# GradientSpaces/LivingScenes

Hardware: AMD Instinct MI355X
Metric: object-instances/sec (encode+match+register), N=1024 pts (higher is better)
Workload: dtype f32 (GEMM products as two-piece f16 splits on the f16 matrix cores, fp32 accumulate: as accurate against fp64 as an fp32 FMA chain)

## Files before the change

### livingscenes_amd/csrc/edge.hip

```cpp
#include "ls_launch.h"
#include "ls_device.h"

namespace ls {

constexpr int EK = 16;

__global__ __launch_bounds__(256) void edge_l0_kernel(const float* __restrict__ pts, const int32_t* __restrict__ knn,
                                                      const float* __restrict__ w0, int N, int Co, float oms,
                                                      float* __restrict__ out, int total) {
    const int lane = threadIdx.x & 63, wave = threadIdx.x >> 6;
    const int sub = lane >> 5, o = lane & 31;
    int pid = (xcd_remap(blockIdx.x, gridDim.x) * 4 + wave) * 2 + sub;
    const bool live = pid < total;
    if (!live) pid = total - 1;
    const int b = pid / N;
    const float* P = pts + (size_t)b * N * 3;
    const float cx = pts[(size_t)pid * 3 + 0], cy = pts[(size_t)pid * 3 + 1], cz = pts[(size_t)pid * 3 + 2];
    const float inv = 1.0f / fmaxf(sqrtf(cx * cx + cy * cy + cz * cz), 1e-12f);
    const float ax = cx * inv, ay = cy * inv, az = cz * inv;
    const int32_t* ki = knn + (size_t)pid * EK;
    __shared__ __attribute__((aligned(16))) float l_edge[4][2][EK][8];
    if (o < EK) {
        const int r = ki[o];
        const float nx = P[(size_t)r * 3 + 0], ny = P[(size_t)r * 3 + 1], nz = P[(size_t)r * 3 + 2];
        float* le = l_edge[wave][sub][o];
        *reinterpret_cast<float4*>(le) = make_float4(ay * nz - az * ny, az * nx - ax * nz, ax * ny - ay * nx, nx - cx);
        *reinterpret_cast<float2*>(le + 4) = make_float2(ny - cy, nz - cz);
    }
    __builtin_amdgcn_s_waitcnt(0xc07f);
    __builtin_amdgcn_wave_barrier();
    for (int c0 = 0; c0 < Co; c0 += 32) {
        const int oc = c0 + o;
        const bool on = oc < Co;
        const int ow = on ? oc : 0;
        const float a0 = w0[0 * Co + ow], a1 = w0[1 * Co + ow], a2 = w0[2 * Co + ow];
        const float d0 = w0[3 * Co + ow], d1 = w0[4 * Co + ow], d2 = w0[5 * Co + ow];
        const float yc0 = a2 * cx, yc1 = a2 * cy, yc2 = a2 * cz, kc0 = d2 * cx, kc1 = d2 * cy, kc2 = d2 * cz;
        float s0 = 0.f, s1 = 0.f, s2 = 0.f;
#pragma unroll 4
        for (int k = 0; k < EK; ++k) {
            const float4 e0 = *reinterpret_cast<const float4*>(l_edge[wave][sub][k]);
            const float2 e1 = *reinterpret_cast<const float2*>(l_edge[wave][sub][k] + 4);
            const float crx = e0.x, cry = e0.y, crz = e0.z, dx = e0.w, dy = e1.x, dz = e1.y;
            float y0 = __builtin_fmaf(a0, crx, __builtin_fmaf(a1, dx, yc0)), y1 = __builtin_fmaf(a0, cry, __builtin_fmaf(a1, dy, yc1)),
                  y2 = __builtin_fmaf(a0, crz, __builtin_fmaf(a1, dz, yc2));
            const float k0 = __builtin_fmaf(d0, crx, __builtin_fmaf(d1, dx, kc0)), k1 = __builtin_fmaf(d0, cry, __builtin_fmaf(d1, dy, kc1)),
                        k2 = __builtin_fmaf(d0, crz, __builtin_fmaf(d1, dz, kc2));
            vn_act(y0, y1, y2, k0, k1, k2, oms);
            s0 += y0; s1 += y1; s2 += y2;
        }
        if (live && on) {
            float* op = out + (size_t)pid * 3 * Co + oc;
            op[0] = s0 * (1.0f / EK); op[Co] = s1 * (1.0f / EK); op[2 * Co] = s2 * (1.0f / EK);
        }
    }
}

__global__ __launch_bounds__(256) void edge_pool_kernel(const float* __restrict__ T, int ldt, const float* __restrict__ Tq, int ldq,
                                                        int NQ, int q_via_rows, const int32_t* __restrict__ knn,
                                                        const int32_t* __restrict__ dst_rows, int Nd, int Ns, int Co,
                                                        float oms, float* __restrict__ out, int total) {
    const int lane = threadIdx.x & 63, wave = threadIdx.x >> 6;
    const int lpp = Co <= 32 ? 32 : 64;
    const int ppw = 64 / lpp;
    const int sub = lane / lpp, ol = lane % lpp;
    int pid = (xcd_remap(blockIdx.x, gridDim.x) * 4 + wave) * ppw + sub;
    const bool live = pid < total;
    if (!live) pid = total - 1;
    const int b = pid / Nd;
    const int drow = (dst_rows && q_via_rows) ? dst_rows[pid] : (pid % Nd);
    const float* Tb = T + (size_t)b * Ns * 3 * ldt;
    const float* Td = Tq + ((size_t)b * NQ + drow) * 3 * ldq;
    const int32_t* ki = knn + (size_t)pid * EK;
    for (int c0 = 0; c0 < Co; c0 += lpp) {
        const int oc = c0 + ol;
        const bool on = oc < Co;
        const int ow = on ? oc : 0;
        float ql[3], qd[3];
#pragma unroll
        for (int x = 0; x < 3; ++x) { ql[x] = Td[x * ldq + ow]; qd[x] = Td[x * ldq + Co + ow]; }
        float s0 = 0.f, s1 = 0.f, s2 = 0.f;
#pragma unroll 4
        for (int k = 0; k < EK; ++k) {
            const float* Tr = Tb + (size_t)ki[k] * 3 * ldt;
            float y0 = Tr[ow] + ql[0], y1 = Tr[ldt + ow] + ql[1], y2 = Tr[2 * ldt + ow] + ql[2];
            const float k0 = Tr[Co + ow] + qd[0], k1 = Tr[ldt + Co + ow] + qd[1], k2 = Tr[2 * ldt + Co + ow] + qd[2];
            vn_act(y0, y1, y2, k0, k1, k2, oms);
            s0 += y0; s1 += y1; s2 += y2;
        }
        if (live && on) {
            float* op = out + (size_t)pid * 3 * Co + oc;
            op[0] = s0 * (1.0f / EK); op[Co] = s1 * (1.0f / EK); op[2 * Co] = s2 * (1.0f / EK);
        }
    }
}

__global__ __launch_bounds__(256) void edge_attn_kernel(const float* __restrict__ T, int ldt, const float* __restrict__ Tq, int ldq,
                                                        int NQ, int q_via_rows, const int32_t* __restrict__ knn,
                                                        const int32_t* __restrict__ dst_rows, int Nd, int Ns, int Co,
                                                        float oms, float inv_sqrt_dk, float* __restrict__ out, int total) {
    extern __shared__ __attribute__((aligned(16))) float smem[];
    const int lane = threadIdx.x & 63, wave = threadIdx.x >> 6;
    const int nh = Co / 16;
    const int per_wave = 3 * Co + 2 * nh * EK;
    float* lq = smem + (size_t)wave * per_wave;
    float* lscore = lq + 3 * Co;
    float* latt = lscore + nh * EK;
    int pid = xcd_remap(blockIdx.x, gridDim.x) * 4 + wave;
    const bool live = pid < total;
    if (!live) pid = total - 1;
    const int b = pid / Nd;
    const int drow = (dst_rows && q_via_rows) ? dst_rows[pid] : (pid % Nd);
    const float* Tb = T + (size_t)b * Ns * 3 * ldt;
    const float* Td = Tq + ((size_t)b * NQ + drow) * 3 * ldq;
    const int32_t* ki = knn + (size_t)pid * EK;
    int nbr[EK];
#pragma unroll
    for (int k = 0; k < EK; ++k) nbr[k] = ki[k];

    float ssq = 0.f;
    for (int c0 = 0; c0 < Co; c0 += 64) {
        const int oc = c0 + lane;
        if (oc < Co) {
            float y0 = Td[4 * Co + oc], y1 = Td[ldq + 4 * Co + oc], y2 = Td[2 * ldq + 4 * Co + oc];
            const float k0 = Td[5 * Co + oc], k1 = Td[ldq + 5 * Co + oc], k2 = Td[2 * ldq + 5 * Co + oc];
            vn_act(y0, y1, y2, k0, k1, k2, oms);
            lq[oc] = y0; lq[Co + oc] = y1; lq[2 * Co + oc] = y2;
            ssq += y0 * y0 + y1 * y1 + y2 * y2;
        }
    }
    const float inv_q = 1.0f / fmaxf(sqrtf(wave_sum(ssq)), 1e-12f);
    __syncthreads();

    float ssk[EK];
#pragma unroll
    for (int k = 0; k < EK; ++k) ssk[k] = 0.f;
    for (int c0 = 0; c0 < Co; c0 += 64) {
        const int oc = c0 + lane;
        const bool on = oc < Co;
        const int ow = on ? oc : 0;
        float ql[3], qd[3], qv[3];
#pragma unroll
        for (int x = 0; x < 3; ++x) {
            ql[x] = Td[x * ldq + 2 * Co + ow];
            qd[x] = Td[x * ldq + 3 * Co + ow];
            qv[x] = lq[x * Co + ow];
        }
#pragma unroll
        for (int k = 0; k < EK; ++k) {
            const float* Tr = Tb + (size_t)nbr[k] * 3 * ldt;
            float y0 = Tr[2 * Co + ow] + ql[0], y1 = Tr[ldt + 2 * Co + ow] + ql[1], y2 = Tr[2 * ldt + 2 * Co + ow] + ql[2];
            const float k0 = Tr[3 * Co + ow] + qd[0], k1 = Tr[ldt + 3 * Co + ow] + qd[1], k2 = Tr[2 * ldt + 3 * Co + ow] + qd[2];
            vn_act(y0, y1, y2, k0, k1, k2, oms);
            float a = y0 * qv[0] + y1 * qv[1] + y2 * qv[2];
            float s2 = y0 * y0 + y1 * y1 + y2 * y2;
            if (!on) { a = 0.f; s2 = 0.f; }
            ssk[k] += s2;
            const float hs = row16_sum(a);
            if (on && (lane & 15) == 0) lscore[(oc >> 4) * EK + k] = hs;
        }
    }
    float my_invk = 0.f;
#pragma unroll
    for (int k = 0; k < EK; ++k) {
        const float f = 1.0f / fmaxf(sqrtf(wave_sum(ssk[k])), 1e-12f);
        if ((lane & 15) == k) my_invk = f;
    }
    __syncthreads();
    for (int e0 = 0; e0 < nh * EK; e0 += 64) {
        const int e = e0 + lane;
        const bool on = e < nh * EK;
        float v = on ? lscore[e] * inv_q * my_invk * inv_sqrt_dk : -INFINITY;
        const float m = row16_max(v);
        const float ex = on ? expf(v - m) : 0.f;
        const float s = row16_sum(ex);
        if (on) latt[e] = ex / s;
    }
    __syncthreads();

    for (int c0 = 0; c0 < Co; c0 += 64) {
        const int oc = c0 + lane;
        const bool on = oc < Co;
        const int ow = on ? oc : 0;
        float ql[3], qd[3];
#pragma unroll
        for (int x = 0; x < 3; ++x) { ql[x] = Td[x * ldq + ow]; qd[x] = Td[x * ldq + Co + ow]; }
        const float* aw = latt + (ow >> 4) * EK;
        float s0 = 0.f, s1 = 0.f, s2 = 0.f;
#pragma unroll
        for (int k = 0; k < EK; ++k) {
            const float* Tr = Tb + (size_t)nbr[k] * 3 * ldt;
            float y0 = Tr[ow] + ql[0], y1 = Tr[ldt + ow] + ql[1], y2 = Tr[2 * ldt + ow] + ql[2];
            const float k0 = Tr[Co + ow] + qd[0], k1 = Tr[ldt + Co + ow] + qd[1], k2 = Tr[2 * ldt + Co + ow] + qd[2];
            vn_act(y0, y1, y2, k0, k1, k2, oms);
            const float w = aw[k];
            s0 += w * y0; s1 += w * y1; s2 += w * y2;
        }
        if (live && on) {
            float* op = out + (size_t)pid * 3 * Co + oc;
            op[0] = s0; op[Co] = s1; op[2 * Co] = s2;
        }
    }
}


template <int LPP>
__global__ __launch_bounds__(256) __attribute__((amdgpu_waves_per_eu(4))) void edge_pool_v4_kernel(const float* __restrict__ T, int ldt, const float* __restrict__ Tq, int ldq, int NQ,
                                                           int q_via_rows, const int32_t* __restrict__ knn, const int32_t* __restrict__ dst_rows,
                                                           int Nd, int Ns, float oms, float* __restrict__ out, int total) {
    constexpr int PPW = 64 / LPP, Co = 4 * LPP;
    const int lane = threadIdx.x & 63, wave = threadIdx.x >> 6;
    const int sub = lane / LPP, ll = lane % LPP;
    int pid = (xcd_remap(blockIdx.x, gridDim.x) * 4 + wave) * PPW + sub;
    const bool live = pid < total;
    if (!live) pid = total - 1;
    const int b = pid / Nd;
    const int drow = (dst_rows && q_via_rows) ? dst_rows[pid] : (pid % Nd);
    const float* Td = Tq + ((size_t)b * NQ + drow) * 3 * ldq;
    const int c4 = ll * 4;
    int nb[EK];
    {
        const int4* kp = reinterpret_cast<const int4*>(knn + (size_t)pid * EK);
#pragma unroll
        for (int u = 0; u < EK / 4; ++u) { const int4 v = kp[u]; nb[4 * u] = v.x; nb[4 * u + 1] = v.y; nb[4 * u + 2] = v.z; nb[4 * u + 3] = v.w; }
    }
    const F43 ql = ld43(Td + c4, ldq), qd = ld43(Td + Co + c4, ldq);
    F43 acc;
    acc.x = acc.y = acc.z = make_float4(0.f, 0.f, 0.f, 0.f);
    const unsigned row_bytes = 3u * (unsigned)ldt * 4u, lane_off = (unsigned)c4 * 4u, inst_row = (unsigned)b * (unsigned)Ns;
    auto ldrow = [&](unsigned off, int col) {
        asm volatile("" : "+v"(off));
        F43 r;
        r.x = *reinterpret_cast<const float4*>(reinterpret_cast<const char*>(T + col) + off);
        r.y = *reinterpret_cast<const float4*>(reinterpret_cast<const char*>(T + ldt + col) + off);
        r.z = *reinterpret_cast<const float4*>(reinterpret_cast<const char*>(T + 2 * ldt + col) + off);
        return r;
    };
    constexpr int DP = 2;
    F43 py[DP], pd[DP];
#pragma unroll
    for (int d = 0; d < DP; ++d) { const unsigned o = __umul24(inst_row + (unsigned)nb[d], row_bytes) + lane_off; py[d] = ldrow(o, 0); pd[d] = ldrow(o, Co); }
#pragma unroll
    for (int k = 0; k < EK; ++k) {
        F43 y = py[k % DP], kd = pd[k % DP];
        if (k + DP < EK) {
            unsigned o = __umul24(inst_row + (unsigned)nb[k + DP], row_bytes) + lane_off;
            py[k % DP] = ldrow(o, 0); pd[k % DP] = ldrow(o, Co);
        }
        asm volatile("" ::: "memory");
        __builtin_amdgcn_sched_barrier(0);
        y = add43(y, ql);
        kd = add43(kd, qd);
        act43(y, kd, oms);
        acc = add43(acc, y);
        asm volatile("" : "+v"(acc.x.x), "+v"(acc.x.y), "+v"(acc.x.z), "+v"(acc.x.w), "+v"(acc.y.x), "+v"(acc.y.y), "+v"(acc.y.z), "+v"(acc.y.w), "+v"(acc.z.x), "+v"(acc.z.y), "+v"(acc.z.z), "+v"(acc.z.w) :: "memory");
        __builtin_amdgcn_sched_barrier(0);
    }
    if (live) {
        float* op = out + (size_t)pid * 3 * Co + c4;
        const float s = 1.0f / EK;
        *reinterpret_cast<float4*>(op) = make_float4(acc.x.x * s, acc.x.y * s, acc.x.z * s, acc.x.w * s);
        *reinterpret_cast<float4*>(op + Co) = make_float4(acc.y.x * s, acc.y.y * s, acc.y.z * s, acc.y.w * s);
        *reinterpret_cast<float4*>(op + 2 * Co) = make_float4(acc.z.x * s, acc.z.y * s, acc.z.z * s, acc.z.w * s);
    }
}

template <int LPP>
__device__ __forceinline__ void attn_colsum(float (*l_score)[256], const float4& ox, const float4& oy, const float4& oz, bool live, int tid, float* __restrict__ cp) {
    constexpr int PPW = 64 / LPP, PW = 4 * PPW, Co = 4 * LPP;
    const float z = live ? 1.f : 0.f;
    l_score[0][tid] = ox.x * z; l_score[1][tid] = ox.y * z; l_score[2][tid] = ox.z * z; l_score[3][tid] = ox.w * z;
    l_score[4][tid] = oy.x * z; l_score[5][tid] = oy.y * z; l_score[6][tid] = oy.z * z; l_score[7][tid] = oy.w * z;
    l_score[8][tid] = oz.x * z; l_score[9][tid] = oz.y * z; l_score[10][tid] = oz.z * z; l_score[11][tid] = oz.w * z;
    __syncthreads();
    for (int col = tid; col < 3 * Co; col += 256) {
        const int ax = col / Co, c = col - ax * Co;
        const float* sp = &l_score[ax * 4 + (c & 3)][c >> 2];
        float a = 0.f;
#pragma unroll
        for (int pw = 0; pw < PW; ++pw) a += sp[(pw / PPW) * 64 + (pw % PPW) * LPP];
        cp[col] = a;
    }
}

template <int LPP, int NCH>
__global__ __launch_bounds__(256) void edge_attn_v4_kernel(const float* __restrict__ T, int ldt, const float* __restrict__ Tq, int ldq,
                                                           int NQ, int q_via_rows, const int32_t* __restrict__ knn,
                                                           const int32_t* __restrict__ dst_rows, int Nd, int Ns, int Co,
                                                           float oms, float inv_sqrt_dk, float* __restrict__ out, int total,
                                                           float* __restrict__ rowmax, float* __restrict__ colsum) {
    constexpr int PPW = 64 / LPP;
    __shared__ float l_score[NCH][EK][256];
    __shared__ float l_ssk[EK][256];
    const int tid = threadIdx.x, lane = tid & 63, wave = tid >> 6;
    const int sub = lane / LPP, ll = lane % LPP;
    int pid = (xcd_remap(blockIdx.x, gridDim.x) * 4 + wave) * PPW + sub;
    const bool live = pid < total;
    if (!live) pid = total - 1;
    const int b = pid / Nd;
    const int drow = (dst_rows && q_via_rows) ? dst_rows[pid] : (pid % Nd);
    const float* Tb = T + (size_t)b * Ns * 3 * ldt;
    const float* Td = Tq + ((size_t)b * NQ + drow) * 3 * ldq;
    const int32_t* ki = knn + (size_t)pid * EK;

    F43 qf[NCH];
    float ssq = 0.f;
#pragma unroll
    for (int ch = 0; ch < NCH; ++ch) {
        const int c4 = (ch * LPP + ll) * 4;
        qf[ch] = ld43(Td + 4 * Co + c4, ldq);
        const F43 kd = ld43(Td + 5 * Co + c4, ldq);
        act43(qf[ch], kd, oms);
        ssq += dot43(qf[ch], qf[ch]);
    }
    const float inv_q = inv_fro(group_sum<LPP>(ssq));

#pragma unroll
    for (int ch = 0; ch < NCH; ++ch) {
        const int c4 = (ch * LPP + ll) * 4;
        const F43 ql = ld43(Td + 2 * Co + c4, ldq), qd = ld43(Td + 3 * Co + c4, ldq);
#pragma unroll 2
        for (int k = 0; k < EK; ++k) {
            const float* Tr = Tb + (size_t)ki[k] * 3 * ldt;
            F43 y = add43(ld43(Tr + 2 * Co + c4, ldt), ql);
            const F43 kd = add43(ld43(Tr + 3 * Co + c4, ldt), qd);
            act43(y, kd, oms);
            const float s2 = dot43(y, y);
            l_ssk[k][tid] = (ch == 0) ? s2 : l_ssk[k][tid] + s2;
            l_score[ch][k][tid] = quad_sum(dot43(y, qf[ch]));
        }
    }
    float mx[NCH], sum[NCH];
#pragma unroll
    for (int ch = 0; ch < NCH; ++ch) { mx[ch] = -INFINITY; sum[ch] = 0.f; }
#pragma unroll 4
    for (int k = 0; k < EK; ++k) {
        const float invk = inv_fro(group_sum<LPP>(l_ssk[k][tid]));
#pragma unroll
        for (int ch = 0; ch < NCH; ++ch) {
            const float v = l_score[ch][k][tid] * inv_q * invk * inv_sqrt_dk;
            l_score[ch][k][tid] = v;
            mx[ch] = fmaxf(mx[ch], v);
        }
    }
#pragma unroll
    for (int ch = 0; ch < NCH; ++ch) {
#pragma unroll 4
        for (int k = 0; k < EK; ++k) {
            const float ex = expf(l_score[ch][k][tid] - mx[ch]);
            l_score[ch][k][tid] = ex;
            sum[ch] += ex;
        }
    }

    float rmx = 0.f, rmy = 0.f, rmz = 0.f;
#pragma unroll
    for (int ch = 0; ch < NCH; ++ch) {
        const int c4 = (ch * LPP + ll) * 4;
        const F43 ql = ld43(Td + c4, ldq), qd = ld43(Td + Co + c4, ldq);
        F43 acc;
        acc.x = acc.y = acc.z = make_float4(0.f, 0.f, 0.f, 0.f);
#pragma unroll 2
        for (int k = 0; k < EK; ++k) {
            const float* Tr = Tb + (size_t)ki[k] * 3 * ldt;
            F43 y = add43(ld43(Tr + c4, ldt), ql);
            const F43 kd = add43(ld43(Tr + Co + c4, ldt), qd);
            act43(y, kd, oms);
            const float w = l_score[ch][k][tid];
            fma43(acc, w, y);
        }
        const float inv = 1.0f / sum[ch];
        const float4 ox = make_float4(acc.x.x * inv, acc.x.y * inv, acc.x.z * inv, acc.x.w * inv);
        const float4 oy = make_float4(acc.y.x * inv, acc.y.y * inv, acc.y.z * inv, acc.y.w * inv);
        const float4 oz = make_float4(acc.z.x * inv, acc.z.y * inv, acc.z.z * inv, acc.z.w * inv);
        if (live) {
            float* op = out + (size_t)pid * 3 * Co + c4;
            *reinterpret_cast<float4*>(op) = ox;
            *reinterpret_cast<float4*>(op + Co) = oy;
            *reinterpret_cast<float4*>(op + 2 * Co) = oz;
        }
        rmx = fmaxf(rmx, amax_f4(ox)); rmy = fmaxf(rmy, amax_f4(oy)); rmz = fmaxf(rmz, amax_f4(oz));
        if constexpr (NCH == 1) {
            if (colsum) attn_colsum<LPP>(l_score[0], ox, oy, oz, live, tid, colsum + (size_t)xcd_remap(blockIdx.x, gridDim.x) * 3 * Co);
        }
    }
    if (rowmax) {
        rmx = group_max<LPP>(rmx); rmy = group_max<LPP>(rmy); rmz = group_max<LPP>(rmz);
        if (live && ll == 0) { float* rp = rowmax + (size_t)pid * 3; rp[0] = rmx; rp[1] = rmy; rp[2] = rmz; }
    }
}


__global__ __launch_bounds__(64) void edge_presplit_wq_kernel(const float* __restrict__ W, int rows, int Cin, int KS, uint4* __restrict__ planes,
                                                               float* __restrict__ winv) {
    const int tile = blockIdx.x / KS, ks = blockIdx.x % KS, lane = threadIdx.x;
    const int n = tile * 32 + (lane & 31), k = ks * 16 + 8 * (lane >> 5);
    const float* wr = W + (size_t)min(n, rows - 1) * Cin;
    float am = 0.f;
    for (int c = 0; c < Cin; ++c) am = fmaxf(am, fabsf(wr[c]));
    float sc, inv;
    pow2_scale(am, sc, inv);
    if (ks == 0 && lane < 32 && n < rows) winv[n] = inv;
    __attribute__((aligned(16))) float v[8];
#pragma unroll
    for (int c = 0; c < 8; ++c) v[c] = wr[k + c] * sc;
    f16x8_t h, l;
    split8_f16(v, h, l);
    planes[((size_t)blockIdx.x * 2) * 64 + lane] = __builtin_bit_cast(uint4, h);
    planes[((size_t)blockIdx.x * 2 + 1) * 64 + lane] = __builtin_bit_cast(uint4, l);
}
static size_t edge_wq_plane_count(int Co, int Cin) { return (size_t)(6 * Co / 32) * (Cin / 16) * 2 * 64; }
size_t edge_wq_planes_bytes(int Co, int Cin) { return edge_wq_plane_count(Co, Cin) * sizeof(uint4) + (size_t)6 * Co * sizeof(float); }
int edge_presplit_wq_launch(const float* Wq, int Co, int Cin, void* planes, hipStream_t st) {
    hipLaunchKernelGGL(edge_presplit_wq_kernel, dim3((6 * Co / 32) * (Cin / 16)), dim3(64), 0, st, Wq, 6 * Co, Cin, Cin / 16, (uint4*)planes,
                       (float*)((uint4*)planes + edge_wq_plane_count(Co, Cin)));
    LS_LAUNCH_CHECK();
    return LS_OK;
}

template <int LPP, int CIN>
__global__ __launch_bounds__(256) __attribute__((amdgpu_waves_per_eu(3))) void edge_attn_fq_kernel(const float* __restrict__ T, int ldt, const float* __restrict__ cur,
                                                           const uint4* __restrict__ Wp, const int32_t* __restrict__ knn,
                                                           const int32_t* __restrict__ dst_rows, int Nd, int Ns, float oms, float inv_sqrt_dk,
                                                           float* __restrict__ out, int total, float* __restrict__ rowmax, float* __restrict__ colsum) {
    constexpr int PPW = 64 / LPP, PW = 4 * PPW, ROWS = 3 * PW, MT = (ROWS + 31) / 32, Co = LPP * 4, SC = 2 * Co, NT = SC / 32, SLD = SC + 4,
                  KS = CIN / 16, ASTR = CIN * 2 + 16;
    static_assert(MT * NT == 8, "two output tiles per wave");
    __shared__ float l_score[EK][256];
    __shared__ __attribute__((aligned(16))) float slab[ROWS * SLD];
    __shared__ __attribute__((aligned(16))) char a_pl[2][MT * 32 * ASTR];
    __shared__ int a_inv[MT * 32];
    const float* __restrict__ winv = reinterpret_cast<const float*>(Wp + (size_t)(6 * Co / 32) * KS * 128);
    const int tid = threadIdx.x, lane = tid & 63, wave = tid >> 6;
    const int sub = lane / LPP, ll = lane % LPP;
    const int pid0 = xcd_remap(blockIdx.x, gridDim.x) * PW;
    const int pwl = wave * PPW + sub;
    int pid = pid0 + pwl;
    const bool live = pid < total;
    if (!live) pid = total - 1;
    const int b = pid / Nd;
    const float* Tb = T + (size_t)b * Ns * 3 * ldt;
    const int32_t* ki = knn + (size_t)pid * EK;
    const int c4 = ll * 4;

    uint4 wfh[2][KS], wfl[2][KS];
    auto qload = [&](int cb) {
        const uint4* wt = Wp + (size_t)(cb / 32) * KS * 128 + lane;
#pragma unroll
        for (int u = 0; u < (MT == 2 ? 1 : 2); ++u) {
            const int nt = MT == 2 ? wave : wave + 4 * u;
#pragma unroll
            for (int ks = 0; ks < KS; ++ks) {
                wfh[u][ks] = wt[((size_t)(nt * KS + ks) * 2) * 64];
                wfl[u][ks] = wt[((size_t)(nt * KS + ks) * 2 + 1) * 64];
            }
        }
    };
    qload(4 * Co);
    for (int c = tid; c < MT * 32 * (CIN / 4); c += 256) {
        const int r = c / (CIN / 4), kq = c - r * (CIN / 4);
        uint2 h = make_uint2(0u, 0u), l = make_uint2(0u, 0u);
        float4 v = make_float4(0.f, 0.f, 0.f, 0.f);
        if (r < ROWS) {
            const int pw = r / 3, x = r - 3 * pw;
            const int pa = min(pid0 + pw, total - 1), ba = pa / Nd;
            const int sp = dst_rows ? dst_rows[pa] : pa - ba * Nd;
            v = *reinterpret_cast<const float4*>(cur + (((size_t)ba * Ns + sp) * 3 + x) * CIN + kq * 4);
        }
        {
            float am = fmaxf(fmaxf(fabsf(v.x), fabsf(v.y)), fmaxf(fabsf(v.z), fabsf(v.w)));
            am = max8(am);
            if constexpr (CIN == 64) am = dpp_max<0x140>(am);
            float sc, inv;
            pow2_scale(am, sc, inv);
            if (kq == 0) a_inv[r] = pow2_e(inv);
            split2_f16_pair(f32x2_t{v.x * sc, v.y * sc}, h.x, l.x);
            split2_f16_pair(f32x2_t{v.z * sc, v.w * sc}, h.y, l.y);
        }
        *reinterpret_cast<uint2*>(&a_pl[0][r * ASTR + kq * 8]) = h;
        *reinterpret_cast<uint2*>(&a_pl[1][r * ASTR + kq * 8]) = l;
    }
    __syncthreads();

    auto qmma = [&](int cb) {
        __builtin_amdgcn_sched_barrier(0);
#pragma unroll
        for (int u = 0; u < 2; ++u) {
            const int mt = MT == 2 ? u : 0, nt = MT == 2 ? wave : wave + 4 * u;
            const int aoff = (32 * mt + (lane & 31)) * ASTR + (lane >> 5) * 16;
            f32x16_t acc;
#pragma unroll
            for (int r = 0; r < 16; ++r) acc[r] = 0.f;
#pragma unroll
            for (int ks = 0; ks < KS; ++ks) {
                const f16x8_t ah = __builtin_bit_cast(f16x8_t, *reinterpret_cast<const uint4*>(&a_pl[0][aoff + ks * 32]));
                const f16x8_t al = __builtin_bit_cast(f16x8_t, *reinterpret_cast<const uint4*>(&a_pl[1][aoff + ks * 32]));
                const f16x8_t bh = __builtin_bit_cast(f16x8_t, wfh[MT == 2 ? 0 : u][ks]);
                const f16x8_t bl = __builtin_bit_cast(f16x8_t, wfl[MT == 2 ? 0 : u][ks]);
                acc = __builtin_amdgcn_mfma_f32_32x32x16_f16(al, bh, acc, 0, 0, 0);
                acc = __builtin_amdgcn_mfma_f32_32x32x16_f16(ah, bh, acc, 0, 0, 0);
                acc = __builtin_amdgcn_mfma_f32_32x32x16_f16(ah, bl, acc, 0, 0, 0);
            }
            const int row0 = 32 * mt + 4 * (lane >> 5);
            float* sp = slab + row0 * SLD + 32 * nt + (lane & 31);
            const int ce = pow2_e(winv[cb + 32 * nt + (lane & 31)]);
#pragma unroll
            for (int r = 0; r < 16; ++r) {
                const int dr = (r & 3) + 8 * (r >> 2);
                if (row0 + dr < ROWS) sp[dr * SLD] = scale_pow2(acc[r], a_inv[row0 + dr] + ce);
            }
        }
    };
    const float* srow = slab + 3 * pwl * SLD + c4;
    auto lds43 = [&](int col) {
        F43 r;
        r.x = *reinterpret_cast<const float4*>(srow + col);
        r.y = *reinterpret_cast<const float4*>(srow + SLD + col);
        r.z = *reinterpret_cast<const float4*>(srow + 2 * SLD + col);
        return r;
    };

    qmma(4 * Co);
    __syncthreads();
    qload(2 * Co);
    F43 qf = lds43(0);
    {
        const F43 kd = lds43(Co);
        act43(qf, kd, oms);
    }
    const float inv_q = inv_fro(group_sum<LPP>(dot43(qf, qf)));
    __syncthreads();

    unsigned nb[EK / 2];
    {
        const int4* kp = reinterpret_cast<const int4*>(ki);
#pragma unroll
        for (int u = 0; u < EK / 4; ++u) { const int4 v = kp[u]; nb[2 * u] = (unsigned)v.x | ((unsigned)v.y << 16); nb[2 * u + 1] = (unsigned)v.z | ((unsigned)v.w << 16); }
    }
    const unsigned row_bytes = 3u * (unsigned)ldt * 4u;
    const unsigned lane_off = (unsigned)c4 * 4u;
    const unsigned inst_row = (unsigned)b * (unsigned)Ns;
    auto noff = [&](int k) { return __umul24(inst_row + ((k & 1) ? nb[k >> 1] >> 16 : nb[k >> 1] & 0xFFFFu), row_bytes) + lane_off; };
    auto ldrow = [&](unsigned off, int col) {
        asm volatile("" : "+v"(off));
        F43 r;
        r.x = *reinterpret_cast<const float4*>(reinterpret_cast<const char*>(T + col) + off);
        r.y = *reinterpret_cast<const float4*>(reinterpret_cast<const char*>(T + ldt + col) + off);
        r.z = *reinterpret_cast<const float4*>(reinterpret_cast<const char*>(T + 2 * ldt + col) + off);
        return r;
    };
    qmma(2 * Co);
    __syncthreads();
    {
        constexpr int DP = 2;
        F43 py[DP], pd[DP];
#pragma unroll
        for (int d = 0; d < DP; ++d) { const unsigned o = noff(d); py[d] = ldrow(o, 2 * Co); pd[d] = ldrow(o, 3 * Co); }
        const F43 ql = lds43(0), qd = lds43(Co);
#pragma unroll
        for (int k = 0; k < EK; ++k) {
            F43 y = py[k % DP], kd = pd[k % DP];
            if (k + DP < EK) { const unsigned o = noff(k + DP); py[k % DP] = ldrow(o, 2 * Co); pd[k % DP] = ldrow(o, 3 * Co); }
            __builtin_amdgcn_sched_barrier(0);
            y = add43(y, ql);
            kd = add43(kd, qd);
            act43(y, kd, oms);
            const float invk = inv_fro(group_sum<LPP>(dot43(y, y)));
            l_score[k][tid] = quad_sum(dot43(y, qf)) * inv_q * invk * inv_sqrt_dk;
            __builtin_amdgcn_sched_barrier(0);
        }
    }
#pragma unroll
    for (int k = 0; k < EK / 2; ++k) asm volatile("" : "+v"(nb[k]));
    __syncthreads();
    qload(0);
    float mx = -INFINITY, sum = 0.f;
#pragma unroll 4
    for (int k = 0; k < EK; ++k) mx = fmaxf(mx, l_score[k][tid]);
#pragma unroll 4
    for (int k = 0; k < EK; ++k) {
        const float ex = expf(l_score[k][tid] - mx);
        l_score[k][tid] = ex;
        sum += ex;
    }
    qmma(0);
    __syncthreads();

    {
        const F43 ql = lds43(0), qd = lds43(Co);
        F43 acc;
        acc.x = acc.y = acc.z = make_float4(0.f, 0.f, 0.f, 0.f);
        constexpr int DP = 2;
        F43 py[DP], pd[DP];
#pragma unroll
        for (int d = 0; d < DP; ++d) { const unsigned o = noff(d); py[d] = ldrow(o, 0); pd[d] = ldrow(o, Co); }
#pragma unroll
        for (int k = 0; k < EK; ++k) {
            F43 y = py[k % DP], kd = pd[k % DP];
            if (k + DP < EK) { const unsigned o = noff(k + DP); py[k % DP] = ldrow(o, 0); pd[k % DP] = ldrow(o, Co); }
            __builtin_amdgcn_sched_barrier(0);
            y = add43(y, ql);
            kd = add43(kd, qd);
            act43(y, kd, oms);
            const float w = l_score[k][tid];
            fma43(acc, w, y);
            __builtin_amdgcn_sched_barrier(0);
        }
        const float inv = 1.0f / sum;
        const float4 ox = make_float4(acc.x.x * inv, acc.x.y * inv, acc.x.z * inv, acc.x.w * inv);
        const float4 oy = make_float4(acc.y.x * inv, acc.y.y * inv, acc.y.z * inv, acc.y.w * inv);
        const float4 oz = make_float4(acc.z.x * inv, acc.z.y * inv, acc.z.z * inv, acc.z.w * inv);
        if (live) {
            float* op = out + (size_t)pid * 3 * Co + c4;
            *reinterpret_cast<float4*>(op) = ox;
            *reinterpret_cast<float4*>(op + Co) = oy;
            *reinterpret_cast<float4*>(op + 2 * Co) = oz;
        }
        if (rowmax) {
            const float rmx = group_max<LPP>(amax_f4(ox)), rmy = group_max<LPP>(amax_f4(oy)), rmz = group_max<LPP>(amax_f4(oz));
            if (live && ll == 0) { float* rp = rowmax + (size_t)pid * 3; rp[0] = rmx; rp[1] = rmy; rp[2] = rmz; }
        }
        if (colsum) attn_colsum<LPP>(l_score, ox, oy, oz, live, tid, colsum + (size_t)(pid0 / PW) * 3 * Co);
    }
}

int edge_l0_launch(const float* pts, const int32_t* knn, const float* w0, int B, int N, int Co, float neg_slope, float* out,
                   hipStream_t st) {
    const int total = B * N;
    hipLaunchKernelGGL(edge_l0_kernel, dim3(cdiv(total, 8)), dim3(256), 0, st, pts, knn, w0, N, Co, 1.0f - neg_slope, out, total);
    LS_LAUNCH_CHECK();
    return LS_OK;
}

int edge_run(const Edge& e, const EdgePlan& p, hipStream_t st) {
    if (p.kernel == EdgeKernel::FT_128 || p.kernel == EdgeKernel::FT_256) return edge_ft_attn_launch(e, p, st);
    const float *T = e.T, *Tq = e.T + p.q_off;
    const int total = e.B * e.Nd, Nd = e.Nd, Ns = e.Ns, Co = e.Co;
    const float oms = 1.0f - e.neg_slope, isd = 1.0f / sqrtf(3.0f * e.head_c);
    float* rowmax = p.rowmax_parts ? e.rowmax : nullptr;
    float* colsum = p.cs_rows ? e.colsum : nullptr;
    const dim3 grid(p.grid), block(p.block);
    LS_REQUIRE(p.kernel < EdgeKernel::ATTN || (e.head_c == 16 && Co % 16 == 0 && p.lds <= 64 * 1024),
               "edge_attn: head width must be 16 and divide Co, Co at most 512 (head_c=%d Co=%d)", e.head_c, Co);
#define LS_POOL(K) hipLaunchKernelGGL(K, grid, block, 0, st, T, p.ldp, Tq, p.ldq, p.NQ, p.qvr, e.knn, e.dst_rows, Nd, Ns, oms, e.out, total)
#define LS_V4(LPP, NCH) hipLaunchKernelGGL((edge_attn_v4_kernel<LPP, NCH>), grid, block, 0, st, T, p.ldp, Tq, p.ldq, p.NQ, p.qvr, e.knn, e.dst_rows, Nd, Ns, Co, oms, isd, e.out, total, rowmax, colsum)
#define LS_FQ(LPP, CIN) hipLaunchKernelGGL((edge_attn_fq_kernel<LPP, CIN>), grid, block, 0, st, T, p.ldp, e.cur, (const uint4*)e.planes, e.knn, e.dst_rows, Nd, Ns, oms, isd, e.out, total, rowmax, colsum)
    switch (p.kernel) {
    case EdgeKernel::ATTN_FQ_16_32: LS_FQ(16, 32); break;
    case EdgeKernel::ATTN_FQ_16_64: LS_FQ(16, 64); break;
    case EdgeKernel::ATTN_FQ_32_64: LS_FQ(32, 64); break;
    case EdgeKernel::POOL_V4_8: LS_POOL(edge_pool_v4_kernel<8>); break;
    case EdgeKernel::POOL_V4_16: LS_POOL(edge_pool_v4_kernel<16>); break;
    case EdgeKernel::POOL:
        hipLaunchKernelGGL(edge_pool_kernel, grid, block, 0, st, T, p.ldp, Tq, p.ldq, p.NQ, p.qvr, e.knn, e.dst_rows, Nd, Ns, Co, oms, e.out, total);
        break;
    case EdgeKernel::ATTN_V4_16: LS_V4(16, 1); break;
    case EdgeKernel::ATTN_V4_32: LS_V4(32, 1); break;
    case EdgeKernel::ATTN_V4_64: LS_V4(64, 1); break;
    case EdgeKernel::ATTN_V4_64X2: LS_V4(64, 2); break;
    case EdgeKernel::ATTN:
        hipLaunchKernelGGL(edge_attn_kernel, grid, block, p.lds, st, T, p.ldp, Tq, p.ldq, p.NQ, p.qvr, e.knn, e.dst_rows, Nd, Ns, Co, oms, isd, e.out, total);
        break;
    default: LS_REQUIRE(false, "edge_run: the plan names no kernel of edge.hip");
    }
#undef LS_POOL
#undef LS_V4
#undef LS_FQ
    LS_LAUNCH_CHECK();
    return LS_OK;
}

}
```

Before: 57080.

## Double-buffer q/k/v slabs in edge attention to overlap GEMMs with gathers

Adds a compile-time two-slab mode, enabled by default for two of the three kernel variants. It computes the query and key projection GEMMs back to back into separate LDS slabs and loads the next weight fragments while the MFMAs are still in flight. The value GEMM is then issued right after the neighbour-row prefetch, which removes several __syncthreads and lets global gathers overlap matrix work. In exchange the kernel uses more LDS for the second slab, which can lower occupancy, and row staging is trimmed to the real row count.

```diff
diff --git a/livingscenes_amd/csrc/edge.hip b/livingscenes_amd/csrc/edge.hip
--- a/livingscenes_amd/csrc/edge.hip
+++ b/livingscenes_amd/csrc/edge.hip
@@ -418,6 +418,11 @@
     return LS_OK;
 }
 
+#ifndef LS_FQ_TWO_SLABS
+#define LS_FQ_TWO_SLABS 6
+#endif
+constexpr bool fq_two_slabs(int LPP, int CIN) { return (LS_FQ_TWO_SLABS >> (LPP == 32 ? 2 : CIN == 64 ? 1 : 0)) & 1; }
+
 template <int LPP, int CIN>
 __global__ __launch_bounds__(256) __attribute__((amdgpu_waves_per_eu(3))) void edge_attn_fq_kernel(const float* __restrict__ T, int ldt, const float* __restrict__ cur,
                                                            const uint4* __restrict__ Wp, const int32_t* __restrict__ knn,
@@ -425,11 +430,14 @@
                                                            float* __restrict__ out, int total, float* __restrict__ rowmax, float* __restrict__ colsum) {
     constexpr int PPW = 64 / LPP, PW = 4 * PPW, ROWS = 3 * PW, MT = (ROWS + 31) / 32, Co = LPP * 4, SC = 2 * Co, NT = SC / 32, SLD = SC + 4,
                   KS = CIN / 16, ASTR = CIN * 2 + 16;
+    constexpr bool TWO = fq_two_slabs(LPP, CIN);
+    constexpr int PR = TWO ? ROWS : MT * 32;
     static_assert(MT * NT == 8, "two output tiles per wave");
+    static_assert(PR * (CIN / 4) % 64 == 0, "whole waves in the staging loop: its DPP row maxima must not meet an inactive lane");
     __shared__ float l_score[EK][256];
-    __shared__ __attribute__((aligned(16))) float slab[ROWS * SLD];
-    __shared__ __attribute__((aligned(16))) char a_pl[2][MT * 32 * ASTR];
-    __shared__ int a_inv[MT * 32];
+    __shared__ __attribute__((aligned(16))) float slab[(TWO ? 2 : 1) * ROWS * SLD];
+    __shared__ __attribute__((aligned(16))) char a_pl[2][PR * ASTR];
+    __shared__ int a_inv[PR];
     const float* __restrict__ winv = reinterpret_cast<const float*>(Wp + (size_t)(6 * Co / 32) * KS * 128);
     const int tid = threadIdx.x, lane = tid & 63, wave = tid >> 6;
     const int sub = lane / LPP, ll = lane % LPP;
@@ -457,7 +465,7 @@
         }
     };
     qload(4 * Co);
-    for (int c = tid; c < MT * 32 * (CIN / 4); c += 256) {
+    for (int c = tid; c < PR * (CIN / 4); c += 256) {
         const int r = c / (CIN / 4), kq = c - r * (CIN / 4);
         uint2 h = make_uint2(0u, 0u), l = make_uint2(0u, 0u);
         float4 v = make_float4(0.f, 0.f, 0.f, 0.f);
@@ -482,50 +490,70 @@
     }
     __syncthreads();
 
-    auto qmma = [&](int cb) {
+    auto qmma = [&](int cb, float* dst, int next_cb = -1) {
         __builtin_amdgcn_sched_barrier(0);
+        f32x16_t acc[2];
+        int ce[2];
+#ifndef LS_FQ_SKIP_QGEMM
 #pragma unroll
         for (int u = 0; u < 2; ++u) {
             const int mt = MT == 2 ? u : 0, nt = MT == 2 ? wave : wave + 4 * u;
-            const int aoff = (32 * mt + (lane & 31)) * ASTR + (lane >> 5) * 16;
-            f32x16_t acc;
-#pragma unroll
-            for (int r = 0; r < 16; ++r) acc[r] = 0.f;
+            const int aoff = min(32 * mt + (lane & 31), PR - 1) * ASTR + (lane >> 5) * 16;
+            ce[u] = pow2_e(winv[cb + 32 * nt + (lane & 31)]);
+#pragma unroll
+            for (int r = 0; r < 16; ++r) acc[u][r] = 0.f;
 #pragma unroll
             for (int ks = 0; ks < KS; ++ks) {
                 const f16x8_t ah = __builtin_bit_cast(f16x8_t, *reinterpret_cast<const uint4*>(&a_pl[0][aoff + ks * 32]));
                 const f16x8_t al = __builtin_bit_cast(f16x8_t, *reinterpret_cast<const uint4*>(&a_pl[1][aoff + ks * 32]));
                 const f16x8_t bh = __builtin_bit_cast(f16x8_t, wfh[MT == 2 ? 0 : u][ks]);
                 const f16x8_t bl = __builtin_bit_cast(f16x8_t, wfl[MT == 2 ? 0 : u][ks]);
-                acc = __builtin_amdgcn_mfma_f32_32x32x16_f16(al, bh, acc, 0, 0, 0);
-                acc = __builtin_amdgcn_mfma_f32_32x32x16_f16(ah, bh, acc, 0, 0, 0);
-                acc = __builtin_amdgcn_mfma_f32_32x32x16_f16(ah, bl, acc, 0, 0, 0);
+                acc[u] = __builtin_amdgcn_mfma_f32_32x32x16_f16(al, bh, acc[u], 0, 0, 0);
+                acc[u] = __builtin_amdgcn_mfma_f32_32x32x16_f16(ah, bh, acc[u], 0, 0, 0);
+                acc[u] = __builtin_amdgcn_mfma_f32_32x32x16_f16(ah, bl, acc[u], 0, 0, 0);
             }
+        }
+#endif
+        if (next_cb >= 0) {
+            __builtin_amdgcn_sched_barrier(0);
+            qload(next_cb);
+            __builtin_amdgcn_sched_barrier(0);
+        }
+#ifndef LS_FQ_SKIP_QGEMM
+#pragma unroll
+        for (int u = 0; u < 2; ++u) {
+            const int mt = MT == 2 ? u : 0, nt = MT == 2 ? wave : wave + 4 * u;
             const int row0 = 32 * mt + 4 * (lane >> 5);
-            float* sp = slab + row0 * SLD + 32 * nt + (lane & 31);
-            const int ce = pow2_e(winv[cb + 32 * nt + (lane & 31)]);
+            float* sp = dst + row0 * SLD + 32 * nt + (lane & 31);
 #pragma unroll
             for (int r = 0; r < 16; ++r) {
                 const int dr = (r & 3) + 8 * (r >> 2);
-                if (row0 + dr < ROWS) sp[dr * SLD] = scale_pow2(acc[r], a_inv[row0 + dr] + ce);
+                if (row0 + dr < ROWS) sp[dr * SLD] = scale_pow2(acc[u][r], a_inv[row0 + dr] + ce[u]);
             }
         }
+#endif
     };
-    const float* srow = slab + 3 * pwl * SLD + c4;
-    auto lds43 = [&](int col) {
+    float* const kslab = slab + (TWO ? ROWS * SLD : 0);
+    const int srow = 3 * pwl * SLD + c4;
+    auto lds43 = [&](const float* sl, int col) {
         F43 r;
-        r.x = *reinterpret_cast<const float4*>(srow + col);
-        r.y = *reinterpret_cast<const float4*>(srow + SLD + col);
-        r.z = *reinterpret_cast<const float4*>(srow + 2 * SLD + col);
+        r.x = *reinterpret_cast<const float4*>(sl + srow + col);
+        r.y = *reinterpret_cast<const float4*>(sl + srow + SLD + col);
+        r.z = *reinterpret_cast<const float4*>(sl + srow + 2 * SLD + col);
         return r;
     };
 
-    qmma(4 * Co);
+    if constexpr (TWO) {
+        qmma(4 * Co, slab, 2 * Co);
+        qmma(2 * Co, kslab);
+    } else {
+        qmma(4 * Co, slab);
+    }
     __syncthreads();
-    qload(2 * Co);
-    F43 qf = lds43(0);
+    qload(TWO ? 0 : 2 * Co);
+    F43 qf = lds43(slab, 0);
     {
-        const F43 kd = lds43(Co);
+        const F43 kd = lds43(slab, Co);
         act43(qf, kd, oms);
     }
     const float inv_q = inv_fro(group_sum<LPP>(dot43(qf, qf)));
@@ -549,14 +577,22 @@
         r.z = *reinterpret_cast<const float4*>(reinterpret_cast<const char*>(T + 2 * ldt + col) + off);
         return r;
     };
-    qmma(2 * Co);
-    __syncthreads();
+    constexpr int DP = 2;
+    F43 py[DP], pd[DP];
+    auto prefetch = [&](int c_lin, int c_dir) {
+#pragma unroll
+        for (int d = 0; d < DP; ++d) { const unsigned o = noff(d); py[d] = ldrow(o, c_lin); pd[d] = ldrow(o, c_dir); }
+    };
+    if constexpr (TWO) {
+        prefetch(2 * Co, 3 * Co);
+        qmma(0, slab);
+    } else {
+        qmma(2 * Co, slab);
+        __syncthreads();
+    }
     {
-        constexpr int DP = 2;
-        F43 py[DP], pd[DP];
-#pragma unroll
-        for (int d = 0; d < DP; ++d) { const unsigned o = noff(d); py[d] = ldrow(o, 2 * Co); pd[d] = ldrow(o, 3 * Co); }
-        const F43 ql = lds43(0), qd = lds43(Co);
+        if constexpr (!TWO) prefetch(2 * Co, 3 * Co);
+        const F43 ql = lds43(kslab, 0), qd = lds43(kslab, Co);
 #pragma unroll
         for (int k = 0; k < EK; ++k) {
             F43 y = py[k % DP], kd = pd[k % DP];
@@ -572,8 +608,9 @@
     }
 #pragma unroll
     for (int k = 0; k < EK / 2; ++k) asm volatile("" : "+v"(nb[k]));
+    if constexpr (TWO) { prefetch(0, Co); __builtin_amdgcn_sched_barrier(0); }
     __syncthreads();
-    qload(0);
+    if constexpr (!TWO) qload(0);
     float mx = -INFINITY, sum = 0.f;
 #pragma unroll 4
     for (int k = 0; k < EK; ++k) mx = fmaxf(mx, l_score[k][tid]);
@@ -583,17 +620,16 @@
         l_score[k][tid] = ex;
         sum += ex;
     }
-    qmma(0);
-    __syncthreads();
+    if constexpr (!TWO) {
+        qmma(0, slab);
+        __syncthreads();
+    }
 
     {
-        const F43 ql = lds43(0), qd = lds43(Co);
+        const F43 ql = lds43(slab, 0), qd = lds43(slab, Co);
         F43 acc;
         acc.x = acc.y = acc.z = make_float4(0.f, 0.f, 0.f, 0.f);
-        constexpr int DP = 2;
-        F43 py[DP], pd[DP];
-#pragma unroll
-        for (int d = 0; d < DP; ++d) { const unsigned o = noff(d); py[d] = ldrow(o, 0); pd[d] = ldrow(o, Co); }
+        if constexpr (!TWO) prefetch(0, Co);
 #pragma unroll
         for (int k = 0; k < EK; ++k) {
             F43 y = py[k % DP], kd = pd[k % DP];
```

Measured after the change: 57270, median of 6. No clear change (+0.3%).
